# YuhuaXu/ImageMosaicing

Hardware: AMD Instinct MI355X
Metric: image-pairs/sec (detect+match+H+warp), 4000x3000 UAV frames (higher is better)
Workload: dtype i16 fixed-point pyramid filtered in f32 (as the reference's OpenCV), f32 (RANSAC / warp coordinates), int8 MFMA with int32 accumulation (descriptor distances, exact), u8 (pixels); 1 GPU; C3: ONE 500-frame 4000x3000 UAV survey, pair window 2 (499 pairs), SIFT(2000,3,0.01,20) + exact BF match + 3x3 grid select + Ransac2D + MosaicImagesRefined warp; frames=500, pairs=499, frames_per_gpu=500, pairs_per_gpu=499

## Files before the change

### imagemosaicing_amd/csrc/sift.hip

```cpp
#include "common.h"
#include "sift_plan.h"
#include <memory>
#include "detmath.h"
#include <cmath>
#include <type_traits>

namespace {

using namespace sift_plan;
constexpr int MAX_INTERP = 5, ORI_BINS = 36;
constexpr int FIXPT_SCALE = 48;
constexpr float DOG_THRESHOLD_P1 = 21.0f;
constexpr float HIST_Q = 1024.0f;
constexpr int SIFT_BATCH_MAX = MI355_SIFT_BATCH_MAX;
static_assert(SIFT_BATCH_MAX == BATCH_MAX, "sift_plan.h: BATCH_MAX");
typedef int16_t lvl_t;

__host__ __device__ __forceinline__ int reflect101(int p, int n) {
    if (n == 1) return 0;
    while (p < 0 || p >= n) { if (p < 0) p = -p; else p = 2 * n - 2 - p; }
    return p;
}

typedef float v2f __attribute__((ext_vector_type(2)));
struct __attribute__((aligned(4))) uint2_a4 { unsigned x, y; };
typedef float v4f __attribute__((ext_vector_type(4)));

__device__ __forceinline__ v4f ld4(const lvl_t* p) {
    const uint2 q = *reinterpret_cast<const uint2*>(p);
    v4f o;
    o.x = (float)(int)(short)(q.x & 0xffffu); o.y = (float)((int)q.x >> 16);
    o.z = (float)(int)(short)(q.y & 0xffffu); o.w = (float)((int)q.y >> 16);
    return o;
}
__device__ __forceinline__ float ld1(const lvl_t* p) { return (float)(int)*p; }
__device__ __forceinline__ int sat16(float v) {
    int q = (int)rintf(v);
    q = q < -32768 ? -32768 : (q > 32767 ? 32767 : q);
    return q;
}
__device__ __forceinline__ float gray48(const uint8_t* p) {
    return (float)(((1868 * (int)p[0] + 9617 * (int)p[1] + 4899 * (int)p[2] + 8192) >> 14) * FIXPT_SCALE);
}

__device__ __forceinline__ int xcd_remap(int bid, int nb) {
    const int q = nb >> 3, r = nb & 7, xcd = bid & 7, local = bid >> 3;
    const int base = xcd < r ? xcd * (q + 1) : r * (q + 1) + (xcd - r) * q;
    return base + local;
}

template <int J, int NPP, class F> __device__ __forceinline__ bool static_rows(F& f) {
    if constexpr (J < NPP) { if (!f(std::integral_constant<int, J>{})) return false; return static_rows<J + 1, NPP>(f); }
    else return true;
}

struct Blur16Args {
    const lvl_t* src;
    const uint8_t* bgr[SIFT_BATCH_MAX];
    int bgr_ws[SIFT_BATCH_MAX];
    lvl_t* dst;
    lvl_t* ds;
    int w, h;
    int tiles_x, tiles_y;
    float k[2 * MAX_R + 1];
    float kp[2 * (MAX_R + 1)];
    size_t fstride;
    int nb;
};

template <int R, bool BGR>
__global__ __launch_bounds__(256) void blur16_tile(Blur16Args a) {
    constexpr int ROWS = T16H + 2 * R, COLS = T16W + 2 * R, PIN = COLS | 1, PMID = T16W + 4;
    __shared__ float s_in[ROWS * PIN];
    __shared__ __attribute__((aligned(16))) float s_mid[ROWS * PMID];
    const int tid = threadIdx.x, fr = blockIdx.y;
    const int tile = xcd_remap(blockIdx.x, a.tiles_x * a.tiles_y);
    const int ty = tile / a.tiles_x, tx = tile - ty * a.tiles_x;
    const int x0 = tx * T16W, y0 = ty * T16H;
    const lvl_t* src = BGR ? nullptr : a.src + (size_t)fr * a.fstride;
    const uint8_t* bgr = a.bgr[0]; int bws = a.bgr_ws[0];
    if (BGR) {
#pragma unroll
        for (int q = 1; q < SIFT_BATCH_MAX; q++) if (fr == q) { bgr = a.bgr[q]; bws = a.bgr_ws[q]; }
    }
// ... 116 lines not shown
__global__ __launch_bounds__(256) __attribute__((amdgpu_waves_per_eu(W, W))) void blur16_stream(Blur16Args a, int L, int nstrip, int nseg) {
    blur16_stream_body<R, BGR, DS>(a, L, nstrip, nseg);
}

__global__ __launch_bounds__(256) void downsample16(const lvl_t* src, int sw, lvl_t* dst, int dw, int dh, size_t fstride) {
    src += (size_t)blockIdx.z * fstride; dst += (size_t)blockIdx.z * fstride;
    const int x = blockIdx.x * 64 + (threadIdx.x & 63), y = blockIdx.y * 4 + (threadIdx.x >> 6);
    if (x < dw && y < dh) dst[(size_t)y * dw + x] = src[(size_t)(2 * y) * sw + 2 * x];
}

struct OctaveDev { lvl_t* lv[N_LEVELS]; int w, h; };

constexpr int ECAP = 128;
constexpr int REG_STRIDE = 32;
struct BatchStride { size_t pyr, claimed, cand, refined, kps, cube, sel, mins; };
struct FrameOuts { mi355_keypoint* kp[SIFT_BATCH_MAX]; uint8_t* d8[SIFT_BATCH_MAX]; };

struct Refined { int o, layer, r, c; float xi, xr, xc, contr, scl; unsigned start; };

struct PyrDev { OctaveDev oc[MAX_OCT]; unsigned* claimed[MAX_OCT]; unsigned* mins[MAX_OCT]; int n_oct; };

__device__ __forceinline__ float dogv(const OctaveDev& oc, size_t foff, int lvl, int r, int c) {
    const size_t o = foff + (size_t)r * oc.w + c;
    return (float)((int)oc.lv[lvl + 1][o] - (int)oc.lv[lvl][o]);
}

__device__ __forceinline__ void solve3(const float a[3][3], const float b[3], float x[3]) {
    const float det = (a[0][0] * (a[1][1] * a[2][2] - a[2][1] * a[1][2]) - a[0][1] * (a[1][0] * a[2][2] - a[2][0] * a[1][2])) + a[0][2] * (a[1][0] * a[2][1] - a[2][0] * a[1][1]);
    if (det == 0.0f) { x[0] = x[1] = x[2] = 0.0f; return; }
    const float d = 1.0f / det;
    x[0] = d * ((b[0] * (a[1][1] * a[2][2] - a[1][2] * a[2][1]) - a[0][1] * (b[1] * a[2][2] - a[1][2] * b[2])) + a[0][2] * (b[1] * a[2][1] - a[1][1] * b[2]));
    x[1] = d * ((a[0][0] * (b[1] * a[2][2] - a[1][2] * b[2]) - b[0] * (a[1][0] * a[2][2] - a[1][2] * a[2][0])) + a[0][2] * (a[1][0] * b[2] - b[1] * a[2][0]));
    x[2] = d * ((a[0][0] * (a[1][1] * b[2] - b[1] * a[2][1]) - a[0][1] * (a[1][0] * b[2] - b[1] * a[2][0])) + b[0] * (a[1][0] * a[2][1] - a[1][1] * a[2][0]));
}

struct FitOff { float xi, xr, xc; };
template <class DV>
__device__ __forceinline__ FitOff fit_step(DV dv, int L, int R, int C) {
    const float img_scale = 1.0f / (float)(255 * FIXPT_SCALE);
    const float deriv_scale = img_scale * 0.5f, second_scale = img_scale, cross_scale = img_scale * 0.25f;
    float dD[3];
    dD[0] = (dv(L, R, C + 1) - dv(L, R, C - 1)) * deriv_scale;
    dD[1] = (dv(L, R + 1, C) - dv(L, R - 1, C)) * deriv_scale;
    dD[2] = (dv(L + 1, R, C) - dv(L - 1, R, C)) * deriv_scale;
    const float v2 = dv(L, R, C) * 2.0f;
    const float dxx = (dv(L, R, C + 1) + dv(L, R, C - 1) - v2) * second_scale;
    const float dyy = (dv(L, R + 1, C) + dv(L, R - 1, C) - v2) * second_scale;
    const float dss = (dv(L + 1, R, C) + dv(L - 1, R, C) - v2) * second_scale;
    const float dxy = (dv(L, R + 1, C + 1) - dv(L, R + 1, C - 1) - dv(L, R - 1, C + 1) + dv(L, R - 1, C - 1)) * cross_scale;
    const float dxs = (dv(L + 1, R, C + 1) - dv(L + 1, R, C - 1) - dv(L - 1, R, C + 1) + dv(L - 1, R, C - 1)) * cross_scale;
    const float dys = (dv(L + 1, R + 1, C) - dv(L + 1, R - 1, C) - dv(L - 1, R + 1, C) + dv(L - 1, R - 1, C)) * cross_scale;
    const float A[3][3] = {{dxx, dxy, dxs}, {dxy, dyy, dys}, {dxs, dys, dss}};
    float X[3];
    solve3(A, dD, X);
    FitOff f; f.xi = -X[2]; f.xr = -X[1]; f.xc = -X[0];
    return f;
}
template <class DV>
__device__ __forceinline__ bool fit_accept(DV dv, int L, int R, int C, FitOff f, float contrast_thr, float edge_thr, float& contr) {
    const float img_scale = 1.0f / (float)(255 * FIXPT_SCALE);
    const float deriv_scale = img_scale * 0.5f, second_scale = img_scale, cross_scale = img_scale * 0.25f;
    float dD0 = (dv(L, R, C + 1) - dv(L, R, C - 1)) * deriv_scale;
    float dD1 = (dv(L, R + 1, C) - dv(L, R - 1, C)) * deriv_scale;
    float dD2 = (dv(L + 1, R, C) - dv(L - 1, R, C)) * deriv_scale;
    const float t = ((0.0f + dD0 * f.xc) + dD1 * f.xr) + dD2 * f.xi;
    contr = dv(L, R, C) * img_scale + t * 0.5f;
    if (fabsf(contr) * (float)N_LAYERS < contrast_thr) return false;
    const float v2 = dv(L, R, C) * 2.0f;
    const float dxx = (dv(L, R, C + 1) + dv(L, R, C - 1) - v2) * second_scale;
    const float dyy = (dv(L, R + 1, C) + dv(L, R - 1, C) - v2) * second_scale;
    const float dxy = (dv(L, R + 1, C + 1) - dv(L, R + 1, C - 1) - dv(L, R - 1, C + 1) + dv(L, R - 1, C - 1)) * cross_scale;
    const float tr = dxx + dyy, det = dxx * dyy - dxy * dxy;
    if (det <= 0.0f || (tr * tr) * edge_thr >= ((edge_thr + 1.0f) * (edge_thr + 1.0f)) * det) return false;
    return true;
}
__device__ __forceinline__ int fit_state(FitOff f) {
    if (fabsf(f.xi) < 0.5f && fabsf(f.xr) < 0.5f && fabsf(f.xc) < 0.5f) return 0;
    if (fabsf(f.xi) > 7.0e8f || fabsf(f.xr) > 7.0e8f || fabsf(f.xc) > 7.0e8f) return 1;
    if (!(f.xi == f.xi) || !(f.xr == f.xr) || !(f.xc == f.xc)) return 1;
    return 2;
}

__global__ __launch_bounds__(256) void extrema_kernel(OctaveDev oc, int octave, unsigned long long* cand, unsigned* count, unsigned cap, unsigned* overflow, BatchStride bs,
                                                      float* cube, unsigned cube_cap) {
    {
        const size_t f = blockIdx.y;
#pragma unroll
        for (int l = 0; l < N_LEVELS; l++) oc.lv[l] += f * bs.pyr;
        cand += f * bs.cand; count += f * CCNT_STRIDE; overflow += f * CNT_STRIDE; cube += f * bs.cube;
    }
    constexpr int PC = EW + 8;
    constexpr int P4 = PC / 4;
    constexpr int RW = EH + 2;
    __shared__ v4f s_d4[5][RW * P4];
    __shared__ unsigned long long s_list[ECAP];
    __shared__ unsigned s_n, s_base;
    const int tid = threadIdx.x;
    const int tiles_x = (oc.w + EW - 1) / EW, tiles_y = (oc.h + EH - 1) / EH;
    const int tile = xcd_remap(blockIdx.x, tiles_x * tiles_y);
    const int tyy = tile / tiles_x, txx = tile - tyy * tiles_x;
    const int x0 = txx * EW, y0 = tyy * EH;
    if (tid == 0) s_n = 0;
    const bool vec = ((oc.w & 3) == 0) && (x0 - 4 >= 0) && (x0 + EW + 4 <= oc.w) && ((reinterpret_cast<uintptr_t>(oc.lv[0]) & 7) == 0);
    if (vec) {
        for (int idx = tid; idx < RW * (EW / 4); idx += 256) {
            const int ry = idx / (EW / 4), c4 = idx - ry * (EW / 4);
            int gy = y0 - 1 + ry;
            gy = gy < 0 ? 0 : (gy > oc.h - 1 ? oc.h - 1 : gy);
            const size_t o = (size_t)gy * oc.w + (x0 + 4 * c4);
            v4f g[N_LEVELS];
#pragma unroll
            for (int l = 0; l < N_LEVELS; l++) g[l] = ld4(oc.lv[l] + o);
#pragma unroll
            for (int l = 0; l < 5; l++) s_d4[l][ry * P4 + 1 + c4] = g[l + 1] - g[l];
        }
        if (tid < 2 * RW) {
            const int ry = tid >> 1, side = tid & 1;
            int gy = y0 - 1 + ry;
            gy = gy < 0 ? 0 : (gy > oc.h - 1 ? oc.h - 1 : gy);
            const size_t o = (size_t)gy * oc.w + (side ? x0 + EW : x0 - 1);
            float g[N_LEVELS];
#pragma unroll
            for (int l = 0; l < N_LEVELS; l++) g[l] = ld1(oc.lv[l] + o);
#pragma unroll
            for (int l = 0; l < 5; l++) reinterpret_cast<float*>(s_d4[l])[ry * PC + (side ? 4 + EW : 3)] = g[l + 1] - g[l];
        }
    } else {
        for (int idx = tid; idx < RW * PC; idx += 256) {
            const int ry = idx / PC, rx = idx - ry * PC;
            int gy = y0 - 1 + ry, gx = x0 - 4 + rx;
            gy = gy < 0 ? 0 : (gy > oc.h - 1 ? oc.h - 1 : gy);
            gx = gx < 0 ? 0 : (gx > oc.w - 1 ? oc.w - 1 : gx);
            const size_t o = (size_t)gy * oc.w + gx;
            float g[N_LEVELS];
#pragma unroll
            for (int l = 0; l < N_LEVELS; l++) g[l] = ld1(oc.lv[l] + o);
#pragma unroll
            for (int l = 0; l < 5; l++) reinterpret_cast<float*>(s_d4[l])[idx] = g[l + 1] - g[l];
        }
    }
    __syncthreads();
    for (int item = tid; item < EH * (EW / 4); item += 256) {
        const int ly = item / (EW / 4), xg = item - ly * (EW / 4);
        const int r = y0 + ly;
        float cm[5][6], cn[5][6], mid[5][6], top[5][6], bot[5][6];
#pragma unroll
        for (int pl = 0; pl < 5; pl++) {
            const float* base = reinterpret_cast<const float*>(s_d4[pl]) + (ly + 1) * PC + 4 * xg + 4;
#pragma unroll
            for (int rr = -1; rr <= 1; rr++) {
                const float* q = base + rr * PC;
                const v4f c4 = *reinterpret_cast<const v4f*>(q);
                float v[6] = {q[-1], c4.x, c4.y, c4.z, c4.w, q[4]};
#pragma unroll
                for (int j = 0; j < 6; j++) { if (rr == -1) top[pl][j] = v[j]; else if (rr == 0) mid[pl][j] = v[j]; else bot[pl][j] = v[j]; }
            }
#pragma unroll
            for (int j = 0; j < 6; j++) {
                cm[pl][j] = fmaxf(fmaxf(top[pl][j], mid[pl][j]), bot[pl][j]);
                cn[pl][j] = fminf(fminf(top[pl][j], mid[pl][j]), bot[pl][j]);
            }
        }
        unsigned hit = 0;
#pragma unroll
        for (int k = 0; k < 4; k++) {
            const int j = k + 1;
#pragma unroll
            for (int layer = 1; layer <= N_LAYERS; layer++) {
                const float val = mid[layer][j];
                float mx = fmaxf(fmaxf(cm[layer - 1][j - 1], cm[layer - 1][j]), cm[layer - 1][j + 1]);
                mx = fmaxf(mx, fmaxf(fmaxf(cm[layer + 1][j - 1], cm[layer + 1][j]), cm[layer + 1][j + 1]));
                mx = fmaxf(mx, fmaxf(fmaxf(cm[layer][j - 1], cm[layer][j + 1]), fmaxf(top[layer][j], bot[layer][j])));
                float mn = fminf(fminf(cn[layer - 1][j - 1], cn[layer - 1][j]), cn[layer - 1][j + 1]);
                mn = fminf(mn, fminf(fminf(cn[layer + 1][j - 1], cn[layer + 1][j]), cn[layer + 1][j + 1]));
                mn = fminf(mn, fminf(fminf(cn[layer][j - 1], cn[layer][j + 1]), fminf(top[layer][j], bot[layer][j])));
                const float q = val > 0.0f ? mx : -mn;
                hit |= fabsf(val) >= fmaxf(q, DOG_THRESHOLD_P1) ? (1u << ((layer - 1) * 4 + k)) : 0u;
            }
        }
        unsigned cmask = 0;
#pragma unroll
        for (int k = 0; k < 4; k++) { const int c = x0 + 4 * xg + k; cmask |= (c >= IMG_BORDER && c < oc.w - IMG_BORDER) ? (0x111u << k) : 0u; }
        hit = (r >= IMG_BORDER && r < oc.h - IMG_BORDER) ? (hit & cmask) : 0u;
        while (hit) {
            const int bb = __builtin_ctz(hit); hit &= hit - 1;
            const int layer = bb / 4 + 1, c = x0 + 4 * xg + (bb & 3);
            const unsigned long long rec = ((unsigned long long)octave << 48) | ((unsigned long long)layer << 40) | ((unsigned long long)r << 20) | (unsigned long long)c;
            const unsigned slot = atomicAdd(&s_n, 1u);
            if (slot < ECAP) s_list[slot] = rec;
            else {
                const unsigned reg = ((unsigned)tile >> REG_SHIFT) & (NREG - 1);
                const unsigned g = atomicAdd(&count[reg * REG_STRIDE], 1u);
                if (g < cap) cand[(size_t)reg * cap + g] = rec; else *overflow = 1;
            }
        }
    }
    __syncthreads();
    const unsigned nloc = s_n < ECAP ? s_n : ECAP;
    const unsigned reg = ((unsigned)tile >> REG_SHIFT) & (NREG - 1);
    if (tid == 0 && nloc) s_base = atomicAdd(&count[reg * REG_STRIDE], nloc);
    __syncthreads();
    for (unsigned i = tid; i < nloc; i += 256) {
        const unsigned g = s_base + i;
        if (g < cap) cand[(size_t)reg * cap + g] = s_list[i] | (g < cube_cap ? (1ull << 63) : 0ull); else *overflow = 1;
    }
    for (unsigned idx = tid; idx < nloc * 27; idx += 256) {
        const unsigned ci = idx / 27, e = idx - ci * 27;
        const unsigned g = s_base + ci;
        if (g >= cube_cap) continue;
        const unsigned long long rec = s_list[ci];
        const int L0 = (int)((rec >> 40) & 0xff), R0 = (int)((rec >> 20) & 0xfffff), C0 = (int)(rec & 0xfffff);
        const int dl = (int)(e / 9) - 1, dr = (int)((e / 3) % 3) - 1, dc = (int)(e % 3) - 1;
        cube[((size_t)reg * 32 + e) * cube_cap + g] = reinterpret_cast<const float*>(s_d4[L0 + dl])[(R0 + dr - y0 + 1) * PC + (C0 + dc - x0) + 4];
    }
}

constexpr int XCAP = 144;
constexpr int XNB_CAP = 64;
constexpr int XRING_DW = 5 * 3 * 128;
constexpr int XNB_DW = 18;
constexpr int XLDS_BYTES = 4 * (XRING_DW * 4 + XCAP * 8 + XNB_CAP * XNB_DW * 4);
static_assert(XWAVES * XLDS_BYTES <= 160 * 1024 && XLDS_BYTES <= 53 * 1024, "extrema_stream: ring + list must leave room for XWAVES workgroups per CU");
typedef short s2 __attribute__((ext_vector_type(2)));
struct XRow { uint2 m[N_LEVELS]; };
struct XDog { s2 m[5][2]; };
__device__ __forceinline__ s2 as_s2(unsigned v) { return __builtin_bit_cast(s2, v); }
__device__ __forceinline__ unsigned as_u(s2 v) { return __builtin_bit_cast(unsigned, v); }
__device__ __forceinline__ s2 pmax(s2 a, s2 b) { return __builtin_elementwise_max(a, b); }
__device__ __forceinline__ s2 pmin(s2 a, s2 b) { return __builtin_elementwise_min(a, b); }
__device__ __forceinline__ unsigned dpp_lower(unsigned v) { return (unsigned)__builtin_amdgcn_update_dpp(0, (int)v, 0x138 , 0xf, 0xf, true); }
__device__ __forceinline__ unsigned dpp_upper(unsigned v) { return (unsigned)__builtin_amdgcn_update_dpp(0, (int)v, 0x130 , 0xf, 0xf, true); }

__device__ __forceinline__ unsigned xtest_row(const XDog& A, const XDog& B, const XDog& C, int xm, int clo, int chi, bool row_ok) {
    s2 hx[5][2], hn[5][2];
#pragma unroll
    for (int p = 0; p < 5; p++) {
        auto h3 = [](s2 c01, s2 c23, bool mx, s2& o01, s2& o23) {
            const unsigned u01 = as_u(c01), u23 = as_u(c23);
            const unsigned l23 = dpp_lower(u23), r01 = dpp_upper(u01);
            const s2 s_m0 = as_s2(__builtin_amdgcn_alignbit(u01, l23, 16));
            const s2 s_12 = as_s2(__builtin_amdgcn_alignbit(u23, u01, 16));
            const s2 s_34 = as_s2(__builtin_amdgcn_alignbit(r01, u23, 16));
            if (mx) { o01 = pmax(pmax(s_m0, c01), s_12); o23 = pmax(pmax(s_12, c23), s_34); }
            else    { o01 = pmin(pmin(s_m0, c01), s_12); o23 = pmin(pmin(s_12, c23), s_34); }
        };
        h3(pmax(pmax(A.m[p][0], B.m[p][0]), C.m[p][0]), pmax(pmax(A.m[p][1], B.m[p][1]), C.m[p][1]), true, hx[p][0], hx[p][1]);
        h3(pmin(pmin(A.m[p][0], B.m[p][0]), C.m[p][0]), pmin(pmin(A.m[p][1], B.m[p][1]), C.m[p][1]), false, hn[p][0], hn[p][1]);
    }
    unsigned hit = 0;
    const s2 t21 = {21, 21}, tm21 = {-21, -21};
#pragma unroll
    for (int layer = 1; layer <= N_LAYERS; layer++) {
#pragma unroll
        for (int r = 0; r < 2; r++) {
            const s2 val = B.m[layer][r];
            const s2 mx = pmax(pmax(pmax(hx[layer - 1][r], hx[layer][r]), hx[layer + 1][r]), t21);
            const s2 mn = pmin(pmin(pmin(hn[layer - 1][r], hn[layer][r]), hn[layer + 1][r]), tm21);
            const bool h0 = (val.x == mx.x) | (val.x == mn.x), h1 = (val.y == mx.y) | (val.y == mn.y);
            hit = (hit << 2) | (h0 ? 2u : 0u) | (h1 ? 1u : 0u);
        }
    }
    if (!row_ok || hit == 0) return 0u;
    unsigned out = 0;
#pragma unroll
    for (int b = 0; b < 12; b++) out |= ((hit >> (11 - b)) & 1u) << b;
    unsigned cmask = 0;
#pragma unroll
    for (int k = 0; k < 4; k++) cmask |= (xm + k >= clo && xm + k < chi) ? (0x111u << k) : 0u;
    return out & cmask;
}

struct XH { s2 hx[5][2], hn[5][2]; };
struct XCen { s2 v[3][2]; };
__device__ __forceinline__ void xrow_extremes(const XDog& d, XH& h, XCen& c) {
#pragma unroll
    for (int p = 0; p < 5; p++) {
        const unsigned u01 = as_u(d.m[p][0]), u23 = as_u(d.m[p][1]);
        const unsigned l23 = dpp_lower(u23), r01 = dpp_upper(u01);
        const s2 s_m0 = as_s2(__builtin_amdgcn_alignbit(u01, l23, 16));
        const s2 s_12 = as_s2(__builtin_amdgcn_alignbit(u23, u01, 16));
        const s2 s_34 = as_s2(__builtin_amdgcn_alignbit(r01, u23, 16));
        h.hx[p][0] = pmax(pmax(s_m0, d.m[p][0]), s_12); h.hx[p][1] = pmax(pmax(s_12, d.m[p][1]), s_34);
        h.hn[p][0] = pmin(pmin(s_m0, d.m[p][0]), s_12); h.hn[p][1] = pmin(pmin(s_12, d.m[p][1]), s_34);
    }
#pragma unroll
    for (int l = 0; l < 3; l++) { c.v[l][0] = d.m[l + 1][0]; c.v[l][1] = d.m[l + 1][1]; }
}
__device__ __forceinline__ unsigned xtest_rows(const XH& A, const XH& B, const XH& C, const XCen& cen, int xm, int clo, int chi, bool row_ok) {
    s2 hx[5][2], hn[5][2];
#pragma unroll
    for (int p = 0; p < 5; p++)
#pragma unroll
        for (int r = 0; r < 2; r++) { hx[p][r] = pmax(pmax(A.hx[p][r], B.hx[p][r]), C.hx[p][r]); hn[p][r] = pmin(pmin(A.hn[p][r], B.hn[p][r]), C.hn[p][r]); }
    unsigned hit = 0;
    const s2 t21 = {21, 21}, tm21 = {-21, -21};
#pragma unroll
    for (int layer = 1; layer <= N_LAYERS; layer++) {
#pragma unroll
        for (int r = 0; r < 2; r++) {
            const s2 val = cen.v[layer - 1][r];
            const s2 mx = pmax(pmax(pmax(hx[layer - 1][r], hx[layer][r]), hx[layer + 1][r]), t21);
            const s2 mn = pmin(pmin(pmin(hn[layer - 1][r], hn[layer][r]), hn[layer + 1][r]), tm21);
            const bool h0 = (val.x == mx.x) | (val.x == mn.x), h1 = (val.y == mx.y) | (val.y == mn.y);
            hit = (hit << 2) | (h0 ? 2u : 0u) | (h1 ? 1u : 0u);
        }
    }
    if (!row_ok || hit == 0) return 0u;
    unsigned out = 0;
#pragma unroll
    for (int b = 0; b < 12; b++) out |= ((hit >> (11 - b)) & 1u) << b;
    unsigned cmask = 0;
#pragma unroll
    for (int k = 0; k < 4; k++) cmask |= (xm + k >= clo && xm + k < chi) ? (0x111u << k) : 0u;
    return out & cmask;
}

__global__ __launch_bounds__(256) __attribute__((amdgpu_waves_per_eu(XWAVES, XWAVES)))
void extrema_stream(OctaveDev oc, int octave, unsigned long long* cand, unsigned* count, unsigned cap, unsigned* overflow, BatchStride bs,
                    float* cube, unsigned cube_cap, int L, int nstrip, int nseg, int nb, int xsw ) {
    const int lane = threadIdx.x & 63, wave = threadIdx.x >> 6;
    int unit = __builtin_amdgcn_readfirstlane(xcd_remap(blockIdx.x, gridDim.x) * 4 + wave);
    const int per = nstrip * nseg, fr = unit / per;
    if (fr >= nb) return;
    unit -= fr * per;
    {
        const size_t f = (size_t)fr;
#pragma unroll
        for (int l = 0; l < N_LEVELS; l++) oc.lv[l] += f * bs.pyr;
        cand += f * bs.cand; count += f * CCNT_STRIDE; overflow += f * CNT_STRIDE; cube += f * bs.cube;
    }
    const int seg = unit / nstrip, strip = unit - seg * nstrip;
    const int xs = strip * xsw, y0 = seg * L;
    const int lact = (oc.h - y0 < L) ? oc.h - y0 : L;
    const unsigned reg = (unsigned)unit & (NREG - 1);
    const int xm = xs - 4 + 4 * lane;
    const int xl = xm < 0 ? 0 : (xm < oc.w - 4 ? xm : oc.w - 4);
    int clo = xs > IMG_BORDER ? xs : IMG_BORDER, chi = xs + xsw < oc.w - IMG_BORDER ? xs + xsw : oc.w - IMG_BORDER;
    if (lane == 0 || lane == 63) { clo = 0; chi = 0; }
    const int hm1 = oc.h - 1;
    auto load_row = [&](int r, XRow& q) {
        r = r < 0 ? 0 : (r > hm1 ? hm1 : r);
        const size_t o = (size_t)r * oc.w + xl;
#pragma unroll
        for (int l = 0; l < N_LEVELS; l++) q.m[l] = *reinterpret_cast<const uint2*>(oc.lv[l] + o);
    };
    auto to_dog = [&](const XRow& q, XDog& d) {
#pragma unroll
        for (int p = 0; p < 5; p++) { d.m[p][0] = as_s2(q.m[p + 1].x) - as_s2(q.m[p].x); d.m[p][1] = as_s2(q.m[p + 1].y) - as_s2(q.m[p].y); }
    };
    __shared__ unsigned s_ring[4][XRING_DW];
    __shared__ unsigned long long s_rec[4][XCAP];
    __shared__ uint2 s_nb[4][XNB_CAP][XNB_DW / 2];
    static_assert(sizeof(s_ring) + sizeof(s_rec) + sizeof(s_nb) == XLDS_BYTES, "XLDS_BYTES");
    auto ring_put = [&](const XDog& d, int slot) {
        unsigned* q = &s_ring[wave][lane * 30 + slot];
#pragma unroll
        for (int p = 0; p < 5; p++) { q[p * 3] = as_u(d.m[p][0]); q[p * 3 + 15] = as_u(d.m[p][1]); }
    };
    int nq = 0;
    auto wave_sync = [&]() { __builtin_amdgcn_fence(__ATOMIC_ACQ_REL, "wavefront"); __builtin_amdgcn_wave_barrier(); };
    auto flush = [&](auto cubes) {
        constexpr bool CUBES = decltype(cubes)::value;
        if (nq == 0) return;
        wave_sync();
        unsigned base = 0;
        if (lane == 0) base = atomicAdd(&count[reg * REG_STRIDE], (unsigned)nq);
        base = __shfl(base, 0);
        for (int idx = lane; idx < nq; idx += 64) {
            const unsigned g = base + (unsigned)idx;
            if (g >= cap) { *overflow = 1; continue; }
            const unsigned long long rec = s_rec[wave][idx];
            const bool has = CUBES && idx < XNB_CAP && g < cube_cap;
            cand[(size_t)reg * cap + g] = rec | (has ? (1ull << 63) : 0ull);
            if (has) {
                const int sh = (rec & 1ull) ? 0 : 16;
                float* cb = cube + (size_t)reg * 32 * cube_cap + g;
#pragma nounroll
                for (int i = 0; i < XNB_DW / 2; i++, cb += (size_t)3 * cube_cap) {
                    const uint2 wv = s_nb[wave][idx][i];
                    const unsigned long long ww = (((unsigned long long)wv.y << 32) | wv.x) >> sh;
                    cb[0] = (float)(int)(short)(ww & 0xffffu);
                    cb[cube_cap] = (float)(int)(short)((ww >> 16) & 0xffffu);
                    cb[(size_t)2 * cube_cap] = (float)(int)(short)((ww >> 32) & 0xffffu);
                }
            }
        }
        wave_sync();
        nq = 0;
    };
    auto emit = [&](unsigned hit, int rc, auto sbc) -> bool {
        constexpr int SB = decltype(sbc)::value;
        constexpr bool IN_LOOP = SB >= 0;
        const int nq0 = nq;
        while (__builtin_amdgcn_ballot_w64(hit != 0)) {
            const bool mine = hit != 0;
            const int bb = mine ? __builtin_ctz(hit) : 0;
            hit &= hit - 1;
            const unsigned long long m = __builtin_amdgcn_ballot_w64(mine);
            const int add = __builtin_popcountll(m);
            if (nq + add > XCAP) {
                if constexpr (IN_LOOP) { nq = nq0; return false; }
                else flush(std::false_type{});
            }
            if constexpr (IN_LOOP) wave_sync();
            if (mine) {
                const int layer = bb / 4 + 1, k = bb & 3, c = xm + k;
                const int slot = nq + __builtin_popcountll(m & ((1ull << lane) - 1ull));
                s_rec[wave][slot] = ((unsigned long long)octave << 48) | ((unsigned long long)layer << 40) | ((unsigned long long)rc << 20) | (unsigned long long)c;
                if (IN_LOOP && slot < XNB_CAP) {
                    const unsigned* q = &s_ring[wave][(2 * lane + ((k + 1) >> 1) - 1) * 15 + (layer - 1) * 3];
                    uint2* nbp = s_nb[wave][slot];
                    uint2 v[XNB_DW / 2];
#pragma unroll
                    for (int pl = 0; pl < 3; pl++)
#pragma unroll
                        for (int dr = 0; dr < 3; dr++) {
                            const int o = pl * 3 + (SB + dr + 2) % 3;
                            v[pl * 3 + dr] = make_uint2(q[o], q[o + 15]);
                        }
#pragma unroll
                    for (int i = 0; i < XNB_DW / 2; i++) nbp[i] = v[i];
                }
            }
            nq += add;
        }
        return true;
    };
    XH win[3];
    XCen cen[3];
    XRow nxt[XD];
    auto prime = [&](int t) {
        XRow q; XDog dq;
        load_row(y0 + t - 1, q); to_dog(q, dq); ring_put(dq, 0); xrow_extremes(dq, win[0], cen[0]);
        load_row(y0 + t, q); to_dog(q, dq); ring_put(dq, 1); xrow_extremes(dq, win[1], cen[1]);
#pragma unroll
        for (int d = 0; d < XD; d++) load_row(y0 + t + 1 + d, nxt[d]);
    };
    prime(0);
    int tb = 0, t_slow = -1;
    for (bool done = false; !done;) {
        for (;;) {
            if (tb >= lact) { done = true; break; }
            if (nq > XNB_CAP / 2) break;
            auto step = [&](auto jc) -> bool {
                constexpr int j = decltype(jc)::value;
                const int tt = tb + j;
                if (tt >= lact) return false;
                const int rc = y0 + tt;
                XH& A = win[j % 3]; XH& B = win[(j + 1) % 3]; XH& Cc = win[(j + 2) % 3];
                { XDog dq; to_dog(nxt[j % XD], dq); ring_put(dq, (j + 2) % 3); xrow_extremes(dq, Cc, cen[(j + 2) % 3]); }
                load_row(rc + 1 + XD, nxt[j % XD]);
                const unsigned hit = xtest_rows(A, B, Cc, cen[(j + 1) % 3], xm, clo, chi, rc >= IMG_BORDER && rc < oc.h - IMG_BORDER);
                if (!emit(hit, rc, std::integral_constant<int, (j + 1) % 3>{})) { t_slow = tt; return false; }
                return true;
            };
            if (!static_rows<0, 3 * XD>(step)) { done = true; break; }
            tb += 3 * XD;
        }
        flush(std::true_type{});
    }
    if (t_slow >= 0) {
        for (int tt = t_slow; tt < lact; tt++) {
            const int rc = y0 + tt;
            XRow q; XDog A, B, Cc;
            load_row(rc - 1, q); to_dog(q, A);
            load_row(rc, q); to_dog(q, B);
            load_row(rc + 1, q); to_dog(q, Cc);
            emit(xtest_row(A, B, Cc, xm, clo, chi, rc >= IMG_BORDER && rc < oc.h - IMG_BORDER), rc, std::integral_constant<int, -1>{});
        }
        flush(std::false_type{});
    }
}

__global__ __launch_bounds__(256) void refine_kernel(PyrDev P, const unsigned long long* cand_all, const unsigned* cand_counts, unsigned cand_cap, unsigned* cand_total,
                                                     float contrast_thr, float edge_thr, float sigma,
                                                     Refined* out, unsigned* out_count, unsigned out_cap, unsigned* out_resp, BatchStride bs,
                                                     const float* cube_all, unsigned cube_cap) {
    const size_t fr = blockIdx.z, foff = fr * bs.pyr;
    cube_all += fr * bs.cube;
    cand_all += fr * bs.cand; cand_counts += fr * CCNT_STRIDE; cand_total += fr * CNT_STRIDE;
    out += fr * bs.refined; out_count += fr * CNT_STRIDE; out_resp += fr * bs.refined;
    const unsigned reg = blockIdx.y;
    unsigned n = cand_counts[reg * REG_STRIDE];
    if (n > cand_cap) n = cand_cap;
    const unsigned long long* cand = cand_all + (size_t)reg * cand_cap;
    if (blockIdx.x == 0 && blockIdx.y == 0 && threadIdx.x < 64) {
        unsigned tot = cand_counts[threadIdx.x * REG_STRIDE];
        for (int off = 32; off > 0; off >>= 1) tot += __shfl_xor(tot, off);
        if (threadIdx.x == 0) cand_total[0] = tot;
    }
    for (unsigned i = blockIdx.x * blockDim.x + threadIdx.x; i < n; i += gridDim.x * blockDim.x) {
        const unsigned long long pk = cand[i];
        const int o = (int)((pk >> 48) & 0xff);
        int L = (int)((pk >> 40) & 0xff), R = (int)((pk >> 20) & 0xfffff), C = (int)(pk & 0xfffff);
        const unsigned start = ((unsigned)L << 28) | ((unsigned)R << 14) | (unsigned)C;
        const OctaveDev& oc = P.oc[o];
        auto dv = [&](int l, int r, int c) { return dogv(oc, foff, l, r, c); };
        FitOff f = {0.0f, 0.0f, 0.0f};
        int it = 0;
        bool alive = true, accepted = false;
        float contr = 0.0f;
        const bool from_cube = (pk >> 63) != 0;
        const bool can_gather = (oc.w & 1) == 0 && (foff & 1) == 0;
        float cv[27];
        auto gather = [&](int l, int r, int c) {
            const int a0 = (c - 1) & ~1, sh = ((c - 1) & 1) * 16;
            int v[4][9];
#pragma unroll
            for (int q = 0; q < 4; q++) {
                const lvl_t* lp = oc.lv[l - 1 + q] + foff;
#pragma unroll
                for (int dr = 0; dr < 3; dr++) {
                    const uint2_a4 wv = *reinterpret_cast<const uint2_a4*>(lp + (size_t)(r - 1 + dr) * oc.w + a0);
                    const unsigned long long ww = (((unsigned long long)wv.y << 32) | wv.x) >> sh;
                    v[q][dr * 3 + 0] = (int)(short)(ww & 0xffffu); v[q][dr * 3 + 1] = (int)(short)((ww >> 16) & 0xffffu); v[q][dr * 3 + 2] = (int)(short)((ww >> 32) & 0xffffu);
                }
            }
#pragma unroll
            for (int dl = 0; dl < 3; dl++)
#pragma unroll
                for (int e = 0; e < 9; e++) cv[dl * 9 + e] = (float)(v[dl + 1][e] - v[dl][e]);
        };
        if (from_cube || can_gather) {
            for (; it < MAX_INTERP; it++) {
                if (it == 0 && from_cube) {
                    const float* cb = cube_all + (size_t)reg * 32 * cube_cap + i;
#pragma unroll
                    for (int e = 0; e < 27; e++) cv[e] = cb[(size_t)e * cube_cap];
                } else if (can_gather) gather(L, R, C);
                else break;
                const int L0 = L, R0 = R, C0 = C;
                auto dvc = [&](int l, int r, int c) { return cv[(l - L0 + 1) * 9 + (r - R0 + 1) * 3 + (c - C0 + 1)]; };
                f = fit_step(dvc, L, R, C);
                const int stt = fit_state(f);
                if (stt == 1) { alive = false; break; }
                if (stt == 0) { accepted = fit_accept(dvc, L, R, C, f, contrast_thr, edge_thr, contr); alive = accepted; break; }
                C += (int)rintf(f.xc); R += (int)rintf(f.xr); L += (int)rintf(f.xi);
                if (L < 1 || L > N_LAYERS || C < IMG_BORDER || C >= oc.w - IMG_BORDER || R < IMG_BORDER || R >= oc.h - IMG_BORDER) { alive = false; break; }
            }
            if (!alive || (can_gather && !accepted)) continue;
        }
        if (!accepted) {
            for (; it < MAX_INTERP; it++) {
                f = fit_step(dv, L, R, C);
                const int stt = fit_state(f);
                if (stt == 0) break;
                if (stt == 1) { alive = false; break; }
                C += (int)rintf(f.xc); R += (int)rintf(f.xr); L += (int)rintf(f.xi);
                if (L < 1 || L > N_LAYERS || C < IMG_BORDER || C >= oc.w - IMG_BORDER || R < IMG_BORDER || R >= oc.h - IMG_BORDER) { alive = false; break; }
            }
            if (!alive || it >= MAX_INTERP) continue;
            if (!fit_accept(dv, L, R, C, f, contrast_thr, edge_thr, contr)) continue;
        }
        const size_t bit = ((size_t)R * oc.w + C) * 4 + (size_t)L;
        const unsigned mask = 1u << (bit & 31);
        if (!P.mins[o]) {
            const unsigned old = atomicOr(&P.claimed[o][fr * bs.claimed + (bit >> 5)], mask);
            if (old & mask) continue;
        }
        const unsigned long long act = __ballot(1);
        const int leader = __builtin_ctzll(act), lane_id = (int)(threadIdx.x & 63);
        unsigned slot = 0;
        if (lane_id == leader) slot = atomicAdd(out_count, (unsigned)__builtin_popcountll(act));
        slot = __shfl(slot, leader) + (unsigned)__builtin_popcountll(act & ((1ull << lane_id) - 1ull));
        if (slot < out_cap) {
            Refined rr;
            rr.o = o; rr.layer = L; rr.r = R; rr.c = C; rr.xi = f.xi; rr.xr = f.xr; rr.xc = f.xc; rr.contr = contr;
            rr.scl = sigma * det_exp2f(((float)L + f.xi) / (float)N_LAYERS);
            rr.start = start;
            out[slot] = rr;
            out_resp[slot] = __float_as_uint(fabsf(contr));
            if (P.mins[o]) atomicMin(&P.mins[o][fr * bs.mins + bit], start);
        } else if (!P.mins[o]) atomicAnd(&P.claimed[o][fr * bs.claimed + (bit >> 5)], ~mask);
    }
}

__device__ __forceinline__ void unclaim_body(const PyrDev& P, const Refined* ref, const unsigned* ref_count, unsigned ref_cap, const BatchStride& bs, size_t fr, unsigned first, unsigned step) {
    ref += fr * bs.refined; ref_count += fr * CNT_STRIDE;
    unsigned n = *ref_count;
    if (n > ref_cap) n = ref_cap;
    for (unsigned i = first; i < n; i += step) {
        const Refined rr = ref[i];
        const size_t bit = ((size_t)rr.r * P.oc[rr.o].w + rr.c) * 4 + (size_t)rr.layer;
        atomicAnd(&P.claimed[rr.o][fr * bs.claimed + (bit >> 5)], ~(1u << (bit & 31)));
    }
}

__global__ __launch_bounds__(256) void keepall_live_kernel(PyrDev P, const Refined* ref, const unsigned* ref_count, unsigned ref_cap, unsigned* ctrl, unsigned* list, BatchStride bs) {
    const size_t fr = blockIdx.y;
    ref += fr * bs.refined; ref_count += fr * CNT_STRIDE; ctrl += fr * CNT_STRIDE; list += fr * bs.refined;
    unsigned n = *ref_count;
    if (n > ref_cap) n = ref_cap;
    const int lane = threadIdx.x & 63;
    for (unsigned i0 = blockIdx.x * blockDim.x; i0 < n; i0 += gridDim.x * blockDim.x) {
        const unsigned i = i0 + threadIdx.x;
        bool take = false;
        if (i < n) {
            const Refined rr = ref[i];
            const size_t bit = ((size_t)rr.r * P.oc[rr.o].w + rr.c) * 4 + (size_t)rr.layer;
            take = P.mins[rr.o][fr * bs.mins + bit] == rr.start;
        }
        const unsigned long long m = __builtin_amdgcn_ballot_w64(take);
        if (m) {
            const int first = __builtin_ctzll(m);
            unsigned base = 0;
            if (lane == first) base = atomicAdd(&ctrl[2], (unsigned)__builtin_popcountll(m));
            base = __shfl(base, first);
            if (take) list[base + (unsigned)__builtin_popcountll(m & ((1ull << lane) - 1ull))] = i;
        }
    }
}
// ... 742 lines not shown
    }
    SiftWork* s = ctx->sift_slots[slot];
    int rc = MI355_OK;
    static const size_t total_mem = [] { size_t fr = 0, tot = 0; return hipMemGetInfo(&fr, &tot) == hipSuccess ? tot : (size_t)0; }();
    const int nb = batch_frames(w, h, keepall, ctx->sift_batch, SIFT_SLOTS, total_mem);
    if (!s->pend.empty() && !(s->lay.same_key(lay) && s->nb == nb)) { rc = sift_run_batch(ctx, s); if (rc != MI355_OK) return rc; }
    rc = sift_prepare(ctx, s, lay, nb);
    if (rc != MI355_OK) return rc;
    auto fit = ctx->feats.find(img_id);
    if (fit != ctx->feats.end() && fit->second.pending) { rc = mi_resolve_features(ctx); if (rc != MI355_OK) return rc; }
    Features& f = ctx->feats[img_id];
    f.w = w; f.h = h;
    MI_HIP(f.kp.reserve(sizeof(mi355_keypoint) * (size_t)(keepall ? kmax : 2048)));
    MI_HIP(f.d8.reserve((size_t)128 * (size_t)(keepall ? kmax : 2048)));
    f.pending = true; f.h_cnt = nullptr; f.ready = nullptr; f.n = 0;
    s->pend.push_back({img_id, d_bgr, ws, ctx->pend_event});
    if ((int)s->pend.size() >= nb) {
        rc = sift_run_batch(ctx, s);
        if (rc != MI355_OK) return rc;
    }
    if (ctx->pinned_used >= PINNED_CHUNK * 64) {
        rc = mi_resolve_features(ctx);
        if (rc != MI355_OK) return rc;
        ctx->pinned_used = 0;
    }
    if (n_kp) {
        rc = mi_resolve_features(ctx);
        if (rc != MI355_OK) return rc;
        *n_kp = f.n;
    }
    return MI355_OK;
}

struct BatchRun {
    mi355_ctx* ctx; SiftWork* s; hipStream_t st;
    std::vector<SiftWork::Pend> pend;
    std::vector<Features*> fs;
    int n;
    unsigned* cnt;
    FrameOuts outs;
    int enqueue_pyramid();
    void enqueue_keypoints();
    int publish_batch();
};

int BatchRun::enqueue_pyramid() {
    const PyramidTaps& taps = pyramid_taps();
    Routes routes = {ctx->blur_stream, ctx->xstream_min_w, ctx->xstream_min_frames, true};
    for (const SiftWork::Pend& p : pend) routes.base_frames_aligned = routes.base_frames_aligned && ((uintptr_t)p.d_bgr & 3) == 0 && (p.ws & 3) == 0 && p.ws >= 3 * s->lay.w;
    for (const Launch& L : pyramid_launches(s->lay, n, routes)) {
        const OctaveDev& oc = s->P.oc[L.octave];
        const dim3 grid(L.gx, L.gy, L.gz), block(256);
        switch (L.kind) {
            case BLUR_STREAM: case BLUR_TILE: {
                const bool base = L.level == 0;
                const Taps& t = base ? taps.base : taps.lv[L.level];
                Blur16Args a; memset(&a, 0, sizeof(a));
                a.w = oc.w; a.h = oc.h; a.tiles_x = (oc.w + T16W - 1) / T16W; a.tiles_y = (oc.h + T16H - 1) / T16H;
                a.fstride = s->bs.pyr; a.nb = n;
                if (base) for (int k = 0; k < n; k++) { a.bgr[k] = pend[k].d_bgr; a.bgr_ws[k] = pend[k].ws; }
                else a.src = oc.lv[L.level - 1];
                a.dst = oc.lv[L.level];
                if (L.ds) a.ds = s->P.oc[L.octave + 1].lv[0];
                memcpy(a.k, t.k, sizeof(float) * (2 * t.r + 1));
                const BlurFn k = base ? blur_kernel<true>(L) : blur_kernel<false>(L);
                if (!k.stream && !k.tile) { ctx->set_error("sift: unsupported kernel radius"); return MI355_ERR_FAILED; }
                ProfScope ps(ctx, k.stream ? "gauss_stream" : "gauss", L.bytes, st);
                if (k.stream) {
                    for (int i = 0; i <= t.r; i++) { a.kp[2 * i] = a.k[i]; a.kp[2 * i + 1] = i ? a.k[i - 1] : 0.0f; }
                    hipLaunchKernelGGL(k.stream, grid, block, 0, st, a, L.L, L.nstrip, L.nseg);
                } else hipLaunchKernelGGL(k.tile, grid, block, 0, st, a);
                break;
            }
            case DOWNSAMPLE: {
                const OctaveDev& pv = s->P.oc[L.octave - 1];
                ProfScope ps(ctx, "downsample", L.bytes, st);
                hipLaunchKernelGGL(downsample16, grid, block, 0, st, pv.lv[N_LAYERS], pv.w, oc.lv[0], oc.w, oc.h, s->bs.pyr);
                break;
            }
            case EXTREMA_STREAM: case EXTREMA_TILE: {
                ProfScope ps(ctx, "extrema", L.bytes, st);
                const SiftBufs& d = s->b;
                if (L.kind == EXTREMA_STREAM) hipLaunchKernelGGL(extrema_stream, grid, block, 0, st, oc, L.octave, d.cand.as<unsigned long long>(), d.ccnt.as<unsigned>(), s->lay.cand_cap, cnt + 4, s->bs,
                                                                 d.cube.as<float>(), s->lay.cube_cap, L.L, L.nstrip, L.nseg, n, L.xsw);
                else hipLaunchKernelGGL(extrema_kernel, grid, block, 0, st, oc, L.octave, d.cand.as<unsigned long long>(), d.ccnt.as<unsigned>(), s->lay.cand_cap, cnt + 4, s->bs, d.cube.as<float>(), s->lay.cube_cap);
                break;
            }
        }
    }
    return MI355_OK;
}

void BatchRun::enqueue_keypoints() {
    const SiftBufs& d = s->b;
    const Layout& lay = s->lay;
    const BatchStride bs = s->bs;
    const unsigned kmax = (unsigned)lay.kmax;
    {
        ProfScope ps(ctx, "refine", 0.0, st);
        hipLaunchKernelGGL(refine_kernel, dim3(REFINE_GX, NREG, n), dim3(256), 0, st, s->P, d.cand.as<unsigned long long>(), d.ccnt.as<unsigned>(), lay.cand_cap, cnt + 0,
                           ctx->p.contrast_threshold, ctx->p.edge_threshold, 1.6f, d.refined.as<Refined>(), cnt + 1, lay.ref_cap, d.rhist.as<unsigned>(), bs, d.cube.as<float>(), lay.cube_cap);
    }
    {
        ProfScope ps(ctx, "kp_select", 0.0, st);
        if (lay.keepall) {
            hipLaunchKernelGGL(keepall_live_kernel, dim3(256, n), dim3(256), 0, st, s->P, d.refined.as<Refined>(), cnt + 1, lay.ref_cap, cnt + 8, d.olist.as<unsigned>(), bs);
            hipLaunchKernelGGL(keepall_reset_kernel, dim3(256, n), dim3(256), 0, st, s->P, d.refined.as<Refined>(), cnt + 1, lay.ref_cap, bs);
        } else {
            hipLaunchKernelGGL(select_unclaim_kernel, dim3(1 + UNCLAIM_WGS, n), dim3(1024), 0, st, s->P, d.refined.as<Refined>(), bs, d.rhist.as<unsigned>(), cnt + 1, lay.ref_cap,
                               (unsigned)ctx->p.nfeatures + 256u, cnt + 8, bs.refined, d.olist.as<unsigned>());
        }
    }
    for (int pass = 0; pass < (lay.keepall ? 1 : 2); pass++) {
        {
            ProfScope ps(ctx, "orient", 0.0, st);
            hipLaunchKernelGGL(orient_kernel, dim3(ctx->num_cu * 4, n), dim3(256), 0, st, s->P, d.refined.as<Refined>(), cnt + 1, lay.ref_cap,
                               d.kps.as<KpRec>(), d.kresp.as<unsigned>(), cnt + 2, lay.kp_cap, cnt + 8, pass, bs, d.olist.as<unsigned>());
        }
        ProfScope ps(ctx, "topk", 0.0, st);
        if (lay.keepall) {
            hipLaunchKernelGGL(keepall_sort_tiles_kernel, dim3((kmax + KA_TILE - 1) / KA_TILE, n), dim3(1024), 0, st, d.kps.as<KpRec>(), cnt + 2, lay.kp_cap, kmax,
                               d.ksort.as<unsigned long long>(), lay.ksort_stride, outs, d.sel.as<SelRec>(), bs);
            hipLaunchKernelGGL(keepall_place_kernel, dim3((kmax + 255) / 256, n), dim3(256), 0, st, d.kps.as<KpRec>(), cnt + 2, lay.kp_cap, kmax,
                               d.ksort.as<const unsigned long long>(), lay.ksort_stride, outs, d.sel.as<SelRec>(), reinterpret_cast<int*>(cnt + 3), reinterpret_cast<int*>(cnt + 4), bs);
        } else {
            hipLaunchKernelGGL(topk_kernel, dim3(n), dim3(1024), 0, st, d.kps.as<KpRec>(), d.kresp.as<unsigned>(), cnt + 2, lay.kp_cap, ctx->p.nfeatures,
                               outs, d.sel.as<SelRec>(), reinterpret_cast<int*>(cnt + 3), reinterpret_cast<int*>(cnt + 4), cnt + 8, pass, bs);
        }
    }
    ProfScope ps(ctx, "describe", 0.0, st);
    hipLaunchKernelGGL(describe_kernel, dim3(((int)bs.sel + 3) / 4, n), dim3(256), 0, st, s->P, d.sel.as<SelRec>(), reinterpret_cast<const int*>(cnt + 3), outs, bs);
}

int BatchRun::publish_batch() {
    const Layout& lay = s->lay;
    { int rc = mi_finish_features_batch(ctx, fs.data(), n, reinterpret_cast<const int*>(cnt + 3), (int)CNT_STRIDE, st, lay.keepall ? lay.kmax : 2048); if (rc != MI355_OK) return rc; }
    if (ctx->pinned_used % PINNED_CHUNK + (size_t)n > PINNED_CHUNK) ctx->pinned_used += PINNED_CHUNK - ctx->pinned_used % PINNED_CHUNK;
    int* h0 = nullptr;
    for (int k = 0; k < n; k++) {
        int* hc = pinned_slot(ctx);
        if (!hc) { ctx->set_error("sift: pinned alloc failed"); return MI355_ERR_NOMEM; }
        if (k == 0) h0 = hc;
        Features& f = *fs[k];
        f.h_cnt = hc; f.pending = true; f.n = 0;
        f.caps[0] = 0xffffffffu; f.caps[1] = lay.ref_cap; f.caps[2] = lay.kp_cap;
        f.kp_limit = lay.keepall ? lay.kmax : 0;
    }
    MI_HIP(hipMemcpy2DAsync(h0, 8 * sizeof(int), cnt, CNT_STRIDE * sizeof(unsigned), 8 * sizeof(unsigned), (size_t)n, hipMemcpyDeviceToHost, st));
    MI_HIP(hipEventRecord(s->done, st));
    if (ctx->batch_events_used >= ctx->batch_events.size()) {
        hipEvent_t e = nullptr;
        MI_HIP(hipEventCreateWithFlags(&e, hipEventDisableTiming));
        ctx->batch_events.push_back(e);
    }
    hipEvent_t e = ctx->batch_events[ctx->batch_events_used++];
    MI_HIP(hipEventRecord(e, st));
    for (int k = 0; k < n; k++) fs[k]->ready = e;
    for (int k = 0; k < n; k++) if (pend[k].ev) MI_HIP(hipEventRecord(pend[k].ev, st));
    return MI355_OK;
}

static int sift_run_batch(mi355_ctx* ctx, SiftWork* s) {
    BatchRun b = {};
    b.ctx = ctx; b.s = s;
    b.pend.swap(s->pend);
    const int n = b.n = (int)b.pend.size();
    if (n == 0) return MI355_OK;
    ctx->sift_next = (ctx->sift_next + 1) % SIFT_SLOTS;
    const hipStream_t st = b.st = s->stream;
    MI_HIP(hipEventRecord(ctx->sift_in_ev, ctx->stream));
    MI_HIP(hipStreamWaitEvent(st, ctx->sift_in_ev, 0));
    const bool serial_heavy = ctx->serial_heavy != 0;
    if (serial_heavy && ctx->heavy_ev_valid) MI_HIP(hipStreamWaitEvent(st, ctx->heavy_ev, 0));
    b.cnt = s->b.counters.as<unsigned>();
    MI_HIP(hipMemsetAsync(b.cnt, 0, (size_t)n * CNT_STRIDE * sizeof(unsigned), st));
    MI_HIP(hipMemsetAsync(s->b.ccnt.p, 0, (size_t)n * CCNT_STRIDE * sizeof(unsigned), st));
    for (int k = 0; k < n; k++) {
        Features* f = &ctx->feats[b.pend[k].img_id];
        b.fs.push_back(f);
        b.outs.kp[k] = f->kp.as<mi355_keypoint>(); b.outs.d8[k] = f->d8.as<uint8_t>();
    }
    { const int rc = b.enqueue_pyramid(); if (rc != MI355_OK) return rc; }
    if (serial_heavy) {
        if (!ctx->heavy_ev) MI_HIP(hipEventCreateWithFlags(&ctx->heavy_ev, hipEventDisableTiming));
// ... 15 lines not shown
```

Baseline: 4062 image-pairs/s.

## Pack candidate 3x3x3 cubes as 64-byte i16 records instead of planar floats

Replaces the planar float cube buffer (27 float planes per region, strided by cube_cap) with one 64-byte record per candidate holding the 27 values as packed int16. The extrema kernels now write each record with four 16-byte stores (the stream kernel repacks the parked neighbourhood in LDS first), and refine loads it with four vector loads. The goal is fewer, coalesced sector-sized transactions and about half the cube traffic. The per-frame cube stride now assumes NREG*cube_cap records fit in the old bs.cube allocation, and the float-to-int16 truncation relies on the DoG values already being integer-valued.

```diff
diff --git a/imagemosaicing_amd/csrc/cand_record.h b/imagemosaicing_amd/csrc/cand_record.h
--- /dev/null
+++ b/imagemosaicing_amd/csrc/cand_record.h
@@ -0,0 +1,79 @@
+#pragma once
+#include <stdint.h>
+
+#ifdef __HIP__
+#define MI_CR_HD __host__ __device__ __forceinline__
+#else
+#define MI_CR_HD inline
+#endif
+
+namespace candrec {
+
+constexpr int N_ELEM = 27;
+constexpr int N_DW = 16;
+constexpr int PARKED_DW = 18;
+
+struct alignas(16) Record { uint32_t w[N_DW]; };
+static_assert(sizeof(Record) == 64, "one record per 64-byte sector");
+
+template <class Get> MI_CR_HD void pack_with(Get get, Record& r) {
+#ifdef __HIP__
+#pragma unroll
+#endif
+    for (int d = 0; d < N_DW; d++) {
+        const uint32_t lo = 2 * d < N_ELEM ? get(2 * d) : 0u, hi = 2 * d + 1 < N_ELEM ? get(2 * d + 1) : 0u;
+        r.w[d] = lo | (hi << 16);
+    }
+}
+
+MI_CR_HD void parked_plane(const uint32_t* p6, unsigned c, uint32_t* e9) {
+    const int sh = (c & 1u) ? 0 : 16;
+#ifdef __HIP__
+#pragma unroll
+#endif
+    for (int row = 0; row < 3; row++) {
+        const uint64_t ww = (((uint64_t)p6[2 * row + 1] << 32) | p6[2 * row]) >> sh;
+        e9[3 * row] = (uint32_t)ww & 0xffffu; e9[3 * row + 1] = (uint32_t)(ww >> 16) & 0xffffu; e9[3 * row + 2] = (uint32_t)(ww >> 32) & 0xffffu;
+    }
+}
+typedef uint16_t __attribute__((may_alias)) elem16_t;
+MI_CR_HD void put_plane(void* rec, int pl, const uint32_t* e9) {
+    elem16_t* q = static_cast<elem16_t*>(rec) + 9 * pl;
+#ifdef __HIP__
+#pragma unroll
+#endif
+    for (int k = 0; k < 9; k++) q[k] = (elem16_t)e9[k];
+}
+MI_CR_HD void put_padding(void* rec) {
+    elem16_t* q = static_cast<elem16_t*>(rec);
+    for (int k = N_ELEM; k < 2 * N_DW; k++) q[k] = 0;
+}
+MI_CR_HD void pack_parked_in_place(uint32_t* p, unsigned c) {
+#ifdef __HIP__
+#pragma nounroll
+#endif
+    for (int pl = 0; pl < 3; pl++) {
+        uint32_t e9[9];
+        parked_plane(p + 6 * pl, c, e9);
+        put_plane(p, pl, e9);
+    }
+    put_padding(p);
+}
+MI_CR_HD void pack_parked(const uint32_t* p, unsigned c, Record& r) {
+    uint32_t e[N_ELEM];
+    for (int pl = 0; pl < 3; pl++) parked_plane(p + 6 * pl, c, e + 9 * pl);
+    pack_with([&](int k) -> uint32_t { return e[k]; }, r);
+}
+
+MI_CR_HD void pack_floats(const float* v, Record& r) {
+    pack_with([&](int e) -> uint32_t { return (uint32_t)(int)v[e] & 0xffffu; }, r);
+}
+
+MI_CR_HD void unpack(const Record& r, float* v) {
+#ifdef __HIP__
+#pragma unroll
+#endif
+    for (int e = 0; e < N_ELEM; e++) v[e] = (float)(int)(short)((r.w[e >> 1] >> (16 * (e & 1))) & 0xffffu);
+}
+
+}
diff --git a/imagemosaicing_amd/csrc/sift.hip b/imagemosaicing_amd/csrc/sift.hip
--- a/imagemosaicing_amd/csrc/sift.hip
+++ b/imagemosaicing_amd/csrc/sift.hip
@@ -1,5 +1,6 @@
 #include "common.h"
 #include "sift_plan.h"
+#include "cand_record.h"
 #include <memory>
 #include "detmath.h"
 #include <cmath>
@@ -282,12 +283,12 @@
 }
 
 __global__ __launch_bounds__(256) void extrema_kernel(OctaveDev oc, int octave, unsigned long long* cand, unsigned* count, unsigned cap, unsigned* overflow, BatchStride bs,
-                                                      float* cube, unsigned cube_cap) {
+                                                      candrec::Record* cube, unsigned cube_cap) {
     {
         const size_t f = blockIdx.y;
 #pragma unroll
         for (int l = 0; l < N_LEVELS; l++) oc.lv[l] += f * bs.pyr;
-        cand += f * bs.cand; count += f * CCNT_STRIDE; overflow += f * CNT_STRIDE; cube += f * bs.cube;
+        cand += f * bs.cand; count += f * CCNT_STRIDE; overflow += f * CNT_STRIDE; cube += f * NREG * cube_cap;
     }
     constexpr int PC = EW + 8;
     constexpr int P4 = PC / 4;
@@ -404,14 +405,25 @@
         const unsigned g = s_base + i;
         if (g < cap) cand[(size_t)reg * cap + g] = s_list[i] | (g < cube_cap ? (1ull << 63) : 0ull); else *overflow = 1;
     }
-    for (unsigned idx = tid; idx < nloc * 27; idx += 256) {
-        const unsigned ci = idx / 27, e = idx - ci * 27;
-        const unsigned g = s_base + ci;
+    for (unsigned i = tid; i < nloc; i += 256) {
+        const unsigned g = s_base + i;
         if (g >= cube_cap) continue;
-        const unsigned long long rec = s_list[ci];
+        const unsigned long long rec = s_list[i];
         const int L0 = (int)((rec >> 40) & 0xff), R0 = (int)((rec >> 20) & 0xfffff), C0 = (int)(rec & 0xfffff);
-        const int dl = (int)(e / 9) - 1, dr = (int)((e / 3) % 3) - 1, dc = (int)(e % 3) - 1;
-        cube[((size_t)reg * 32 + e) * cube_cap + g] = reinterpret_cast<const float*>(s_d4[L0 + dl])[(R0 + dr - y0 + 1) * PC + (C0 + dc - x0) + 4];
+        float v[candrec::N_ELEM];
+#pragma unroll
+        for (int dl = 0; dl < 3; dl++)
+#pragma unroll
+            for (int dr = 0; dr < 3; dr++) {
+                const float* q = reinterpret_cast<const float*>(s_d4[L0 - 1 + dl]) + (R0 + dr - y0) * PC + (C0 - x0) + 3;
+#pragma unroll
+                for (int dc = 0; dc < 3; dc++) v[dl * 9 + dr * 3 + dc] = q[dc];
+            }
+        candrec::Record r;
+        candrec::pack_floats(v, r);
+        uint4* dst = reinterpret_cast<uint4*>(cube + (size_t)reg * cube_cap + g);
+#pragma unroll
+        for (int k = 0; k < 4; k++) dst[k] = make_uint4(r.w[4 * k], r.w[4 * k + 1], r.w[4 * k + 2], r.w[4 * k + 3]);
     }
 }
 
@@ -517,7 +529,7 @@
 
 __global__ __launch_bounds__(256) __attribute__((amdgpu_waves_per_eu(XWAVES, XWAVES)))
 void extrema_stream(OctaveDev oc, int octave, unsigned long long* cand, unsigned* count, unsigned cap, unsigned* overflow, BatchStride bs,
-                    float* cube, unsigned cube_cap, int L, int nstrip, int nseg, int nb, int xsw ) {
+                    candrec::Record* cube, unsigned cube_cap, int L, int nstrip, int nseg, int nb, int xsw ) {
     const int lane = threadIdx.x & 63, wave = threadIdx.x >> 6;
     int unit = __builtin_amdgcn_readfirstlane(xcd_remap(blockIdx.x, gridDim.x) * 4 + wave);
     const int per = nstrip * nseg, fr = unit / per;
@@ -527,7 +539,7 @@
         const size_t f = (size_t)fr;
 #pragma unroll
         for (int l = 0; l < N_LEVELS; l++) oc.lv[l] += f * bs.pyr;
-        cand += f * bs.cand; count += f * CCNT_STRIDE; overflow += f * CNT_STRIDE; cube += f * bs.cube;
+        cand += f * bs.cand; count += f * CCNT_STRIDE; overflow += f * CNT_STRIDE; cube += f * NREG * cube_cap;
     }
     const int seg = unit / nstrip, strip = unit - seg * nstrip;
     const int xs = strip * xsw, y0 = seg * L;
@@ -562,27 +574,28 @@
     auto flush = [&](auto cubes) {
         constexpr bool CUBES = decltype(cubes)::value;
         if (nq == 0) return;
+        int fl = lane;
+        asm volatile("" : "+v"(fl));
         wave_sync();
         unsigned base = 0;
-        if (lane == 0) base = atomicAdd(&count[reg * REG_STRIDE], (unsigned)nq);
+        if (fl == 0) base = atomicAdd(&count[reg * REG_STRIDE], (unsigned)nq);
         base = __shfl(base, 0);
-        for (int idx = lane; idx < nq; idx += 64) {
+        for (int idx = fl; idx < nq; idx += 64) {
             const unsigned g = base + (unsigned)idx;
             if (g >= cap) { *overflow = 1; continue; }
-            const unsigned long long rec = s_rec[wave][idx];
             const bool has = CUBES && idx < XNB_CAP && g < cube_cap;
-            cand[(size_t)reg * cap + g] = rec | (has ? (1ull << 63) : 0ull);
-            if (has) {
-                const int sh = (rec & 1ull) ? 0 : 16;
-                float* cb = cube + (size_t)reg * 32 * cube_cap + g;
-#pragma nounroll
-                for (int i = 0; i < XNB_DW / 2; i++, cb += (size_t)3 * cube_cap) {
-                    const uint2 wv = s_nb[wave][idx][i];
-                    const unsigned long long ww = (((unsigned long long)wv.y << 32) | wv.x) >> sh;
-                    cb[0] = (float)(int)(short)(ww & 0xffffu);
-                    cb[cube_cap] = (float)(int)(short)((ww >> 16) & 0xffffu);
-                    cb[(size_t)2 * cube_cap] = (float)(int)(short)((ww >> 32) & 0xffffu);
-                }
+            cand[(size_t)reg * cap + g] = s_rec[wave][idx] | (has ? (1ull << 63) : 0ull);
+        }
+        if constexpr (CUBES) {
+            static_assert(XNB_CAP <= 64 && sizeof(candrec::Record) <= XNB_DW * 4, "a lane per parked candidate; a record fits over its parked form");
+            const int nc = nq < XNB_CAP ? nq : XNB_CAP;
+            if (fl < nc) candrec::pack_parked_in_place(reinterpret_cast<unsigned*>(s_nb[wave][fl]), (unsigned)s_rec[wave][fl]);
+            wave_sync();
+            uint4* dst = reinterpret_cast<uint4*>(cube + (size_t)reg * cube_cap + base);
+            for (int q = fl; q < nc * 4; q += 64) {
+                const uint2* src = &s_nb[wave][q >> 2][(q & 3) * 2];
+                const uint2 a = src[0], b = src[1];
+                if (base + (unsigned)(q >> 2) < cube_cap) dst[q] = make_uint4(a.x, a.y, b.x, b.y);
             }
         }
         wave_sync();
@@ -675,9 +688,9 @@
 __global__ __launch_bounds__(256) void refine_kernel(PyrDev P, const unsigned long long* cand_all, const unsigned* cand_counts, unsigned cand_cap, unsigned* cand_total,
                                                      float contrast_thr, float edge_thr, float sigma,
                                                      Refined* out, unsigned* out_count, unsigned out_cap, unsigned* out_resp, BatchStride bs,
-                                                     const float* cube_all, unsigned cube_cap) {
+                                                     const candrec::Record* cube_all, unsigned cube_cap) {
     const size_t fr = blockIdx.z, foff = fr * bs.pyr;
-    cube_all += fr * bs.cube;
+    cube_all += fr * NREG * cube_cap;
     cand_all += fr * bs.cand; cand_counts += fr * CCNT_STRIDE; cand_total += fr * CNT_STRIDE;
     out += fr * bs.refined; out_count += fr * CNT_STRIDE; out_resp += fr * bs.refined;
     const unsigned reg = blockIdx.y;
@@ -724,9 +737,11 @@
         if (from_cube || can_gather) {
             for (; it < MAX_INTERP; it++) {
                 if (it == 0 && from_cube) {
-                    const float* cb = cube_all + (size_t)reg * 32 * cube_cap + i;
-#pragma unroll
-                    for (int e = 0; e < 27; e++) cv[e] = cb[(size_t)e * cube_cap];
+                    const uint4* cb = reinterpret_cast<const uint4*>(cube_all + (size_t)reg * cube_cap + i);
+                    candrec::Record rc;
+#pragma unroll
+                    for (int k = 0; k < 4; k++) { const uint4 q = cb[k]; rc.w[4 * k] = q.x; rc.w[4 * k + 1] = q.y; rc.w[4 * k + 2] = q.z; rc.w[4 * k + 3] = q.w; }
+                    candrec::unpack(rc, cv);
                 } else if (can_gather) gather(L, R, C);
                 else break;
                 const int L0 = L, R0 = R, C0 = C;
@@ -1635,8 +1650,8 @@
                 ProfScope ps(ctx, "extrema", L.bytes, st);
                 const SiftBufs& d = s->b;
                 if (L.kind == EXTREMA_STREAM) hipLaunchKernelGGL(extrema_stream, grid, block, 0, st, oc, L.octave, d.cand.as<unsigned long long>(), d.ccnt.as<unsigned>(), s->lay.cand_cap, cnt + 4, s->bs,
-                                                                 d.cube.as<float>(), s->lay.cube_cap, L.L, L.nstrip, L.nseg, n, L.xsw);
-                else hipLaunchKernelGGL(extrema_kernel, grid, block, 0, st, oc, L.octave, d.cand.as<unsigned long long>(), d.ccnt.as<unsigned>(), s->lay.cand_cap, cnt + 4, s->bs, d.cube.as<float>(), s->lay.cube_cap);
+                                                                 d.cube.as<candrec::Record>(), s->lay.cube_cap, L.L, L.nstrip, L.nseg, n, L.xsw);
+                else hipLaunchKernelGGL(extrema_kernel, grid, block, 0, st, oc, L.octave, d.cand.as<unsigned long long>(), d.ccnt.as<unsigned>(), s->lay.cand_cap, cnt + 4, s->bs, d.cube.as<candrec::Record>(), s->lay.cube_cap);
                 break;
             }
         }
@@ -1652,7 +1667,7 @@
     {
         ProfScope ps(ctx, "refine", 0.0, st);
         hipLaunchKernelGGL(refine_kernel, dim3(REFINE_GX, NREG, n), dim3(256), 0, st, s->P, d.cand.as<unsigned long long>(), d.ccnt.as<unsigned>(), lay.cand_cap, cnt + 0,
-                           ctx->p.contrast_threshold, ctx->p.edge_threshold, 1.6f, d.refined.as<Refined>(), cnt + 1, lay.ref_cap, d.rhist.as<unsigned>(), bs, d.cube.as<float>(), lay.cube_cap);
+                           ctx->p.contrast_threshold, ctx->p.edge_threshold, 1.6f, d.refined.as<Refined>(), cnt + 1, lay.ref_cap, d.rhist.as<unsigned>(), bs, d.cube.as<candrec::Record>(), lay.cube_cap);
     }
     {
         ProfScope ps(ctx, "kp_select", 0.0, st);
```

After: 4056 image-pairs/s. About the same (-0.1%).
